# ghazalehnt/RecBole

Measured on AMD Instinct MI355X. Metric: train positives/sec (+neg) per node, higher is better.
Workload: dtype fp32; 1 GPU; C2 BPR-MF ml-20m-shape: 138,494 users x 26,745 items (incl. PAD), ~20M interactions RO_RS 0.8/0.1/0.1, embedding 128, 4 uniform negatives, 512 positives (2,048 rows) per step, dense Adam; global_batch=512, per_gpu_batch=512, train_interactions=16014928, parallelism=single, exchange_graph=True, sampler=walk (bit-exact)

## Files before the change

### include/mirec.h

```cpp
#ifndef MIREC_H
#define MIREC_H

#include <stddef.h>
#include <stdint.h>

#ifdef __cplusplus
extern "C" {
#endif

#define MIREC_ABI_VERSION 24

int mirec_abi_version(void);
const char* mirec_last_error(void);

size_t mirec_sample_walk_workspace_size(int64_t batch_keys, int64_t num);
int mirec_sample_walk(const int32_t* random_list, int64_t L, int64_t* pr_dev,
                      const int64_t* keys, int64_t n_keys, int64_t batch_keys,
                      int64_t n_batches, int64_t num,
                      const int64_t* used_ptr, const int32_t* used_cols,
                      const uint32_t* used_bits, int64_t n_bits,
                      int64_t n_key_space, int reject,
                      int64_t* out, int64_t out_stride, int32_t* status_dev,
                      void* ws, size_t ws_bytes, void* stream);

int mirec_sample_walk_segments(const int32_t* random_list, int64_t L, int64_t* pr_dev,
// ... 227 lines not shown
                                const uint32_t* const* masks, const int32_t* want,
                                const int32_t* rows_per_wave, int32_t walk_waves,
                                const float* step_consts_dev, const int32_t* step_base_dev,
                                int32_t step_off, double beta1, double beta2, double eps,
                                double weight_decay, void* stream);
int mirec_row_bitmap(const int64_t* keys, int64_t n_keys, int64_t n_rows, uint32_t* bitmap,
                     void* stream);
#define MIREC_FIRST_NOT_READ (-1)
int mirec_first_read(const int32_t* uniq, const int32_t* n_uniq, int64_t n_batches, int64_t per,
                     int64_t n_rows, int32_t* first, void* stream);
int mirec_adam_flush_first_f32(const mirec_adam_table* tables, int32_t n_tables, int32_t d,
                               const int32_t* const* first, const int32_t* rows_per_wave,
                               const float* step_consts_dev, const int32_t* step_base_dev,
                               int32_t step_off, double beta1, double beta2, double eps,
                               double weight_decay, void* stream);
int mirec_bpr_adam_step_f32(const mirec_adam_table* tables, const int64_t* n_max_uniq,
                            int32_t d, const int64_t* items, int64_t Bc, int32_t T, float gamma,
                            float grad_scale, float* loss_k, const int32_t* u_rec,
                            const int32_t* u_crec, const int32_t* i_rec, const int32_t* i_crec,
                            float* u_part, int32_t* u_join, float* i_part, int32_t* i_join,
                            const float* step_consts_dev, const int32_t* step_base_dev,
                            int32_t step_off, double beta1, double beta2, double eps,
                            double weight_decay, void* stream);
int mirec_step_records(const int64_t* user_keys, const int64_t* item_keys, int64_t n_batches,
                       int64_t Bc, int32_t T, int64_t n_users, int64_t n_items,
                       const int32_t* u_perm, const int32_t* u_uniq, const int32_t* u_seg,
                       const int32_t* u_nu, const int32_t* i_perm, const int32_t* i_uniq,
                       const int32_t* i_seg, const int32_t* i_nu, int32_t* u_rec,
                       int32_t* u_crec, int32_t* i_rec, int32_t* i_crec, int32_t* u_ahead,
                       int32_t* u_nah, int32_t* i_ahead, int32_t* i_nah, void* stream);
// ... 376 lines not shown
```

### recbole_amd/_native.py

```python
from __future__ import annotations

import ctypes
import os
from ctypes import c_double, c_float, c_int, c_int32, c_int64, c_size_t, c_void_p, c_char_p

import torch

_HERE = os.path.dirname(os.path.abspath(__file__))
LIB_PATH = os.environ.get("MIREC_LIB", os.path.join(_HERE, "_lib", "libmirec.so"))

_P = c_void_p


class RowsRef(ctypes.Structure):
    _fields_ = [('lo', _P), ('hi', _P), ('split', c_int64)]


class RowsLd(ctypes.Structure):
    _fields_ = [('lo', _P), ('hi', _P), ('split', c_int64), ('ld', c_int64)]


class SpmmEpilogue(ctypes.Structure):
    _fields_ = [('add', RowsRef), ('add_scale', c_float), ('y', RowsRef), ('acc_in', RowsRef),
                ('acc_out', RowsRef), ('acc_scale', c_float)]
# ... 170 lines not shown
                                             c_int32, c_double, c_double, c_double, c_double,
                                             _P]),
    "mirec_adam_flush_f32": (c_int, [ctypes.POINTER(AdamTable), c_int32, c_int32, _P, _P,
                                     c_int32, c_double, c_double, c_double, c_double, _P]),
    "mirec_adam_flush_rows_f32": (c_int, [ctypes.POINTER(AdamTable), c_int32, c_int32, _P, _P,
                                          _P, c_int32, c_double, c_double, c_double, c_double,
                                          _P]),
    "mirec_adam_flush_masked_f32": (c_int, [ctypes.POINTER(AdamTable), c_int32, c_int32, _P, _P,
                                            _P, c_int32, _P, _P, c_int32, c_double, c_double,
                                            c_double, c_double, _P]),
    "mirec_row_bitmap": (c_int, [_P, c_int64, c_int64, _P, _P]),
    "mirec_first_read": (c_int, [_P, _P, c_int64, c_int64, c_int64, _P, _P]),
    "mirec_adam_flush_first_f32": (c_int, [ctypes.POINTER(AdamTable), c_int32, c_int32, _P, _P,
                                           _P, _P, c_int32, c_double, c_double, c_double,
                                           c_double, _P]),
    "mirec_bpr_adam_step_f32": (c_int, [ctypes.POINTER(AdamTable), _P, c_int32, _P, c_int64,
                                        c_int32, ctypes.c_float, ctypes.c_float, _P, _P, _P,
                                        _P, _P, _P, _P, _P, _P, _P, _P, c_int32, c_double,
                                        c_double, c_double, c_double, _P]),
    "mirec_step_record_ints": (c_int64, [c_int64]),
    "mirec_colsum_multi_f32": (c_int, [_P, _P, _P, _P, c_int32, _P]),
    "mirec_offset_keys": (c_int, [_P, _P, c_int32, c_int64, _P, _P]),
    "mirec_bpr_fwd_bwd_at_ids_f32": (c_int, [_P, c_int64, c_int32, _P, _P, _P, c_int64, c_int32,
                                             ctypes.c_float, ctypes.c_float, _P, _P, _P]),
    "mirec_chunk_group_fits": (c_int, [c_int64, c_int32, c_int64, c_int64, c_int32]),
    "mirec_chunk_group": (c_int, [_P, _P, c_int64, c_int64, c_int32, c_int64, c_int64] + [_P] * 16
                          + [_P]),
    "mirec_step_records": (c_int, [_P, _P, c_int64, c_int64, c_int32, c_int64, c_int64, _P, _P,
                                   _P, _P, _P, _P, _P, _P, _P, _P, _P, _P, _P, _P, _P, _P,
                                   _P]),
# ... 95 lines not shown
                                      _P, _P, _P]),
    "mirec_ngcf_grid_cap": (c_int32, [c_int32]),
    "mirec_ngcf_shape_ok": (c_int, [c_int32, c_int32]),
    "mirec_ngcf_layer_fwd_f32": (c_int, [ctypes.POINTER(RowsLd), _P, c_int64, c_int32, c_int32,
                                         _P, _P, _P, _P, ctypes.POINTER(RowsLd), _P, _P, c_float,
                                         ctypes.c_uint64, _P, _P, _P]),
    "mirec_ngcf_layer_bwd_f32": (c_int, [ctypes.POINTER(RowsLd), ctypes.POINTER(RowsLd), _P,
                                         c_int64, c_int32, c_int32, _P, _P,
                                         ctypes.POINTER(RowsLd), _P, ctypes.POINTER(RowsLd), _P,
                                         _P, _P, c_float, ctypes.c_uint64, _P, _P, _P]),
    "mirec_ngcf_wgrad_splits": (c_int32, [c_int64]),
    "mirec_ngcf_wgrad_f32": (c_int, [_P, ctypes.POINTER(RowsLd), _P, c_int64, c_int32, c_int32,
                                     _P, _P]),
}

ABI_VERSION = 24


class NativeError(RuntimeError):
    pass


_lib = None


def lib():
    global _lib
    if _lib is not None:
        return _lib
    if not os.path.exists(LIB_PATH):
        raise NativeError(
# ... 32 lines not shown
```

### recbole_amd/csrc/adam.hip

```cpp

#include "adam_core.h"

namespace mirec {

template <int D>
__global__ __launch_bounds__(kAdamThreads) void adam_multi_kernel(
    const AdamTables tabs, const float* __restrict__ consts, const int32_t* __restrict__ step_base,
    int step_off, AdamConsts k) {
  constexpr int VPR = D / 4;
  constexpr int RPP = kAdamThreads / VPR;
  static_assert(kAdamThreads % VPR == 0, "row width");
  __shared__ int32_t slot[kAdamRows];
  __shared__ int32_t s_range[2];

  const int si = segment_of(tabs, blockIdx.x);
  const mirec_adam_table& T = tabs.t[si];
  float* __restrict__ P = T.p;
  float* __restrict__ M = T.m;
  float* __restrict__ V = T.v;
  const int32_t* __restrict__ uniq = T.uniq;

  const int64_t lo = ((int64_t)blockIdx.x - tabs.block_start[si]) * kAdamRows;
  const int64_t hi = min(T.n_rows, lo + kAdamRows);
  if (threadIdx.x < kAdamRows) slot[threadIdx.x] = -1;
// ... 261 lines not shown
    const int f = ff.first[si][r0 + lane];
    if (f > kFirstNotRead) {
      target = base + f;
      raw = T.last[r0 + lane];
    }
  }
  uint64_t todo = __ballot(min(raw, target) < target);
  while (todo) {
    const int i = __builtin_ctzll(todo);
    todo &= todo - 1;
    flush_row<D>(T, r0 + i, __builtin_amdgcn_readfirstlane(__shfl(raw, i, 64)),
                 __builtin_amdgcn_readfirstlane(__shfl(target, i, 64)), lane, consts, k);
  }
}

constexpr int kWalkRows = 32;

template <int D>
__global__ __launch_bounds__(64) void adam_flush_walk_kernel(
    const AdamTables tabs, const float* __restrict__ consts, const int32_t* __restrict__ step_base,
    int step_off, AdamConsts k, FlushMasks masks) {
  const int lane = threadIdx.x;
  const int target = step_base[0] + step_off;
  for (int si = 0; si < tabs.n_seg; ++si) {
    const mirec_adam_table& T = tabs.t[si];
    const uint32_t* __restrict__ bits = masks.bits[si];
    const uint32_t flip = masks.want[si] ? 0u : ~0u;
    const int64_t groups = (T.n_rows + kWalkRows - 1) / kWalkRows;
    for (int64_t g = blockIdx.x; g < groups; g += gridDim.x) {
      const int64_t r0 = g * kWalkRows;
      const uint32_t sel = bits ? (bits[g] ^ flip) : ~0u;
      int raw = kZeroState;
      if (lane < kWalkRows && r0 + lane < T.n_rows && ((sel >> lane) & 1u))
        raw = T.last[r0 + lane];
      uint64_t todo = __ballot(flush_needs(T, raw, target));
      while (todo) {
        const int i = __builtin_ctzll(todo);
        todo &= todo - 1;
        flush_row<D>(T, r0 + i, __shfl(raw, i, 64), target, lane, consts, k);
      }
    }
  }
}

}

using namespace mirec;

namespace {

enum class Sched { kStreamed, kDeferred, kFlush, kDeferredPair };

int launch_adam(Sched sched, const mirec_adam_table* tables, int32_t n_tables,
                const int64_t* n_max_uniq, int32_t d, const float* consts,
                const int32_t* step_base, int32_t step_off, double beta1, double beta2,
// ... 36 lines not shown
        set_error("%s: rows per wave %d of table %d not in [1, 64]", what, flush_rows[q], q);
        return -1;
      }
      fr.r[q] = flush_rows[q];
    }
    scan = true;
  }
  const bool walk = masks && walk_waves > 0;
  if (masks && (sched != Sched::kFlush || d < 64 || (!scan && !walk))) {
    set_error("%s: a masked flush needs d >= 64 and rows per wave or a wave count", what);
    return -1;
  }
  FlushMasks fm;
  memset(&fm, 0, sizeof(fm));
  if (masks) fm = *masks;
  if (firsts && (sched != Sched::kFlush || !scan || masks)) {
    set_error("%s: per-row targets need the flush with rows per wave and no mask", what);
    return -1;
  }
  FlushFirst ff;
  memset(&ff, 0, sizeof(ff));
  if (firsts) ff = *firsts;
  int scan_threads = kAdamThreads;
  if (scan && !walk) {
    int64_t waves = 0;
    for (int q = 0; q < n_tables; ++q)
      if (tables[q].n_rows > 0) waves += (tables[q].n_rows + fr.r[q] - 1) / fr.r[q];
    if (waves <= kScanOneWaveMax) scan_threads = 64;
  }
  AdamTables tabs;
  memset(&tabs, 0, sizeof(tabs));
  const bool deferred = sched == Sched::kDeferred;
// ... 48 lines not shown
    }
  }
  (void)VPR;
  for (int q = tabs.n_seg; q <= 2 * kMaxTables; ++q) tabs.block_start[q] = blocks;
  if (blocks == 0) return 0;
  AdamConsts k;
  k.omb1 = (float)(1.0 - beta1);
  k.omb1m1 = k.omb1 - 1.0f;
  k.lerp_small = fabsf(k.omb1) < 0.5f;
  k.b2 = (float)beta2;
  k.omb2 = (float)(1.0 - beta2);
  k.eps = (float)eps;
  k.wd = (float)weight_decay;
  const dim3 grd((unsigned)blocks), blk(kAdamThreads);
  hipStream_t st = (hipStream_t)stream;
#define MIREC_ADAM_SCHED(DD)                                                                 \
  case DD:                                                                                   \
    if (sched == Sched::kStreamed)                                                           \
      hipLaunchKernelGGL(adam_multi_kernel<DD>, grd, blk, 0, st, tabs, consts, step_base,    \
                         step_off, k);                                                       \
    else if (deferred && pair)                                                               \
      hipLaunchKernelGGL((dvec == 2 ? adam_deferred_pair_kernel<DD, float2>                  \
                                    : adam_deferred_pair_kernel<DD, float>),                 \
                         grd, dim3(deferred_block(1)), 0, st, tabs, consts, step_base,       \
                         step_off, k);                                                       \
    else if (deferred)                                                                       \
      hipLaunchKernelGGL((dvec == 4 ? adam_deferred_kernel<DD, float4>                       \
                          : dvec == 2 ? adam_deferred_kernel<DD, float2>                     \
                                      : adam_deferred_kernel<DD, float>),                    \
                         grd, dim3(deferred_block(DD / dvec)), 0, st, tabs, consts,          \
                         step_base, step_off, k);                                            \
    else if (DD >= 64 && walk)                                                               \
      hipLaunchKernelGGL(adam_flush_walk_kernel<(DD >= 64 ? DD : 64)>, grd, dim3(64), 0, st,   \
                         tabs, consts, step_base, step_off, k, fm);                          \
    else if (DD >= 64 && scan && firsts)                                                     \
      hipLaunchKernelGGL(adam_flush_first_kernel<(DD >= 64 ? DD : 64)>, grd,                 \
                         dim3(scan_threads), 0, st, tabs, consts, step_base, step_off, k,    \
                         fr, ff);                                                            \
    else if (DD >= 64 && scan && masks)                                                      \
      hipLaunchKernelGGL((adam_flush_scan_kernel<(DD >= 64 ? DD : 64), true>), grd,          \
                         dim3(scan_threads), 0, st, tabs, consts, step_base, step_off, k,    \
                         fr, fm);                                                            \
    else if (DD >= 64 && scan)                                                               \
      hipLaunchKernelGGL((adam_flush_scan_kernel<(DD >= 64 ? DD : 64), false>), grd,         \
                         dim3(scan_threads), 0, st, tabs, consts, step_base, step_off, k,    \
                         fr, fm);                                                            \
    else if (DD >= 64)                                                                       \
      hipLaunchKernelGGL(adam_flush_row_kernel<(DD >= 64 ? DD : 64)>, grd,                   \
                         dim3(kFlushRowThreads), 0, st, tabs,                                \
// ... 144 lines not shown
  FlushFirst ff;
  memset(&ff, 0, sizeof(ff));
  int n = 0;
  for (int q = 0; q < n_tables; ++q) {
    if (!first[q]) continue;
    sel[n] = tables[q];
    rows[n] = rows_per_wave[q];
    ff.first[n] = first[q];
    ++n;
  }
  if (n == 0) return 0;
  return launch_adam(Sched::kFlush, sel, n, nullptr, d, step_consts_dev, step_base_dev, step_off,
                     beta1, beta2, eps, weight_decay, stream, what, rows, nullptr, 0, &ff);
}

extern "C" int mirec_adam_sparse_grad_f32(float* p, float* m, float* v, int64_t n_rows,
                                          int32_t d, const float* rows, const int32_t* perm,
                                          const int32_t* uniq, const int32_t* seg,
                                          const int32_t* n_uniq_dev, int64_t n_max_uniq,
                                          const float* dense_grad, const float* step_consts_dev,
                                          const int32_t* step_idx_dev, double beta1,
                                          double beta2, double eps, double weight_decay,
                                          void* stream) {
  (void)n_max_uniq;
  if (n_rows == 0) return 0;
  mirec_adam_table t;
  memset(&t, 0, sizeof(t));
  t.p = p; t.m = m; t.v = v; t.n_rows = n_rows;
  t.rows = rows; t.perm = perm; t.uniq = uniq; t.seg = seg; t.n_uniq = n_uniq_dev;
  t.dense_grad = dense_grad;
// ... 152 lines not shown
```

### recbole_amd/csrc/common.h

```cpp
#pragma once
#include <hip/hip_runtime.h>
#include <stdint.h>
#include <stdio.h>
#include <string.h>
#include "../../include/mirec.h"

namespace mirec {

void set_error(const char* fmt, ...);

inline int hip_status(hipError_t e, const char* what) {
  if (e == hipSuccess) return 0;
  set_error("%s: %s", what, hipGetErrorString(e));
  return -(1000 + (int)e);
}

inline int launch_status(const char* what) {
  return hip_status(hipGetLastError(), what);
}

constexpr int kMaxDev = 16;

inline int current_device() {
  int dev = -1;
// ... 25 lines not shown
  if (rc) return rc;
  int n = 1;
  if (per_cu) {
    if (hipOccupancyMaxActiveBlocksPerMultiprocessor(&n, (const void*)kern, threads, lds) !=
        hipSuccess) {
      (void)hipGetLastError();
      n = 1;
    }
    n = n < 1 ? 1 : (n > 4 ? 4 : n);
    *per_cu = n;
  }
  if (dev >= 0) cache[dev] = n;
  return 0;
}

constexpr int kWave = 64;

__device__ __forceinline__ float wave_sum(float x) {
#pragma unroll
  for (int off = 32; off > 0; off >>= 1) x += __shfl_xor(x, off, 64);
  return x;
}

__device__ __forceinline__ int wave_sum_i(int x) {
#pragma unroll
  for (int off = 32; off > 0; off >>= 1) x += __shfl_xor(x, off, 64);
  return x;
}

__device__ __forceinline__ int wave_inclusive_scan(int v) {
// ... 42 lines not shown
```

### recbole_amd/ops.py

```python
from __future__ import annotations

import ctypes

import numpy as np
import torch

from recbole_amd._native import NativeError, check, lib, ptr, stream_handle

KERNEL_EVENTS = None


class timed_launch(object):

    def __init__(self, name):
        self.name = name
        self.ev = None

    def __enter__(self):
        if KERNEL_EVENTS is not None and self.name in KERNEL_EVENTS:
            self.ev = (torch.cuda.Event(enable_timing=True), torch.cuda.Event(enable_timing=True))
            self.ev[0].record()
        return self

    def __exit__(self, *exc):
# ... 769 lines not shown
        nm = (ctypes.c_int64 * len(tables))(*n_max_uniq)
        rc = lib().mirec_adam_deferred_f32(tables, len(tables), nm, d, *args)
    elif schedule == "deferred_pair":
        nm = (ctypes.c_int64 * 2)(*n_max_uniq)
        rc = lib().mirec_adam_deferred_pair_f32(tables, nm, d, *args)
    elif schedule == "flush" and flush_rows is not None:
        rpw = (ctypes.c_int32 * len(tables))(*flush_rows)
        rc = lib().mirec_adam_flush_rows_f32(tables, len(tables), d, rpw, *args)
    elif schedule == "flush":
        rc = lib().mirec_adam_flush_f32(tables, len(tables), d, *args)
    else:
        raise ValueError(f"unknown schedule {schedule!r}")
    check(rc, f"adam_multi[{schedule}]")


_TICKETS = {}


def finish_ticket(device, tag=''):
    key = (str(device), tag)
    t = _TICKETS.get(key)
    if t is None:
        t = _TICKETS[key] = torch.zeros(1, dtype=torch.int32, device=device)
    return t


def chunk_finish(loss_k, n: int, stride: int, n_steps: int, denom: float, loss_hist, step_base):
    _dev(loss_k, torch.float32, "loss_k")
    _dev(step_base, torch.int32, "step_base")
    rc = lib().mirec_chunk_finish(ptr(loss_k), n, stride, n_steps, float(denom), ptr(loss_hist),
# ... 710 lines not shown
```

### recbole_amd/trainer/chunk_plan.py

```python
from __future__ import annotations

import bisect
import math


def plan_chunks(n, Bg, C, ramp, cuts=(), ramps=(0,)):
    full = n // Bg
    bounds = sorted({0, full} | {int(c) for c in cuts if 0 < int(c) < full})
    ramp_at = {int(r) for r in ramps}
    out = []
    for lo, hi in zip(bounds[:-1], bounds[1:]):
        ri = 0 if lo in ramp_at else len(ramp)
        b0 = lo
        while b0 < hi:
            size = ramp[ri] if ri < len(ramp) else C
            ri += 1
            nb = min(size, C, hi - b0)
            out.append((b0, nb, Bg))
            b0 += nb
    if n % Bg:
        out.append((full, 1, n % Bg))
    return out


# ... 49 lines not shown
    on = bool(enabled and fused_step and use_graph and adam_mode == 'deferred')
    return [bool(on and Bc == Bg and nb >= min_steps) for _, nb, Bc in plan]


def advance_rows(nb, Bg, times, n_rows, max_rows):
    out = []
    for per, rows in zip((Bg, (1 + times) * Bg), n_rows):
        frac = min(1.0, nb * per / max(rows, 1))
        r = 1
        while r * 2 <= max_rows and r * 2 * frac <= 1.0:
            r *= 2
        out.append(r)
    return tuple(out)


def chunk_of(plan, b):
    return max(bisect.bisect_right(plan, (b, math.inf)) - 1, 0)
```

### recbole_amd/trainer/fused.py

```python
from __future__ import annotations

import ctypes
import math
import os
from types import SimpleNamespace

import numpy as np
import torch

from recbole_amd import ops
from recbole_amd._native import AdamTable, ChunkPrep, check, lib
from recbole_amd.trainer import chunk_plan
from recbole_amd.trainer.exchange import ExchangeLayout

REC_CONTRIB = 8
ADAM_MODES = ('deferred', 'streamed')


_PREP_STREAMS = {}


def _prep_streams_for(dev, n=2):
    key = (str(dev), n)
    got = _PREP_STREAMS.get(key)
# ... 43 lines not shown
    def __init__(self, C, B, T, G, dev, ahead, tab=None):
        Bg = G * B
        KI = (1 + T) * Bg
        self.user_keys = torch.empty(C * Bg, dtype=torch.int64, device=dev)
        self.item_keys = torch.empty(C * KI, dtype=torch.int64, device=dev)
        self.lu = self.li = None
        if G > 1:
            self.lu = torch.empty(C * B, dtype=torch.int64, device=dev)
            self.li = torch.empty(C * (1 + T) * B, dtype=torch.int64, device=dev)
        self.tab = tab or [_Lists(C, per, dev, ahead) for per in (Bg, KI)]
        self.records = None
        self.bitmap = None
        self.first = None
        self.bg_done = None
        self.bg_busy = False
        self.prep = None
        self.ready, self.walked, self.free = (torch.cuda.Event() for _ in range(3))
        cur = torch.cuda.current_stream(dev)
        for ev in (self.ready, self.walked, self.free):
            ev.record(cur)
        self.free_recorded = False
        self.group_pending = False
        self.ready_on_model = False
        self.chunk = None
        self.graphs = {}


class FusedBPRTrainStep(object):

    CHUNK = 64
    SLOTS = 3
    RAMP = (8, 16, 32)
    FLUSH_EVERY = 64
    FLUSH_SPARSE_MAX_ROWS = 8
    MAIN_FIRST = os.environ.get('MIREC_MAIN_FIRST', '1') != '0'
    SPEC_WALK = os.environ.get('MIREC_SPEC_WALK', '1') != '0'
    BG_FLUSH = os.environ.get('MIREC_BG_FLUSH', '1') != '0'
    BG_WAVES = int(os.environ.get('MIREC_BG_WAVES', '1536'))
    BG_MIN_STEPS = 32
    CHUNK_ADVANCE = os.environ.get('MIREC_CHUNK_ADVANCE', '1') != '0'
    ADV_MIN_STEPS = 32

    def __init__(self, model, optimizer, train_data, chunk=None, use_graph=True,
                 adam_mode='deferred', dist=None, fused_step=None):
        if adam_mode not in ADAM_MODES:
            raise ValueError(f'adam_mode must be one of {ADAM_MODES}, got {adam_mode!r}')
        self.model = model
        self.opt = optimizer
        self.data = train_data
        (self.pU, self.nU), (self.pI, self.nI) = model.fused_embedding_tables()
        self.device = self.pU.device
        self.B = train_data.step
        self.times = train_data.times
        self.uid_field = train_data.uid_field
        self.iid_field = train_data.iid_field
        self.C = chunk or self.CHUNK
# ... 28 lines not shown
        self.loss_hist = torch.zeros(1, dtype=torch.float32, device=dev)
        self.consts = torch.zeros(4, dtype=torch.float32, device=dev)
        self.step_idx = torch.zeros(1, dtype=torch.int32, device=dev)
        self.ticket = torch.zeros(1, dtype=torch.int32, device=dev)
        self.kernel_events = None
        self.kernel_uniq = []
        self.n_eager_steps = 0
        self._rec_w = {}
        self._spec_buf = self._spec_stats = None
        self._gs_R = self._gs = None
        self._users = self._items = None
        self.n_batches = 0
        self._plan, self._flags, self._flush_at = [], [], set()
        self._bg = []
        self._adv = []
        self._bg_pending = None
        self._bg_mark = torch.cuda.Event()
        self._bg_mark.record(torch.cuda.current_stream(dev))
        self._busy0 = None
        self._batches_enqueued = 0
        self._current = True
        self._next_chunk = self._next_group = self._prep_limit = 0
        self._cur = None
        self._last_walked = None
        self._deferred_waits = []
        self._urgent = False
        self._late_top_up = None
        self.opt._ensure_state(self.pU)
        self.opt._ensure_state(self.pI)
        self._tables = (AdamTable * 2)()
# ... 12 lines not shown
        if deferred:
            self.lastU = torch.zeros(self.nU, dtype=torch.int32, device=dev)
            self.lastI = torch.zeros(self.nI, dtype=torch.int32, device=dev)
        self.pU_alt = torch.empty_like(self.pU.data) if self.fused_step else None
        self.pI_alt = torch.empty_like(self.pI.data) if self.fused_step else None
        self._step_scratch = None
        if self.fused_step:
            for sl in self.slots:
                sl.records = [torch.empty(self.C * w, dtype=torch.int32, device=dev)
                              for w in self._rec_ints(self.Bg)]
                sl.bitmap = torch.zeros((self.nU + 31) // 32, dtype=torch.int32, device=dev)
                sl.first = [torch.full((n,), -1, dtype=torch.int32, device=dev)
                            for n in (self.nU, self.nI)]
                sl.bg_done = torch.cuda.Event()
                sl.bg_done.record(torch.cuda.current_stream(dev))
            self._step_scratch = ops.step_scratch(self.Bg, T, d, dev)
        self._n_max = (ctypes.c_int64 * 2)(self.Bg, (1 + T) * self.Bg)
        self._fill_tables()

    def _flush_rows(self, b_end):
        return chunk_plan.flush_rows(b_end, self.Bg, self.times, self.adam_mode, self.d,
                                     [t.n_rows for t in self._tables], self._busy0,
                                     self.FLUSH_SPARSE_MAX_ROWS)

    def _chunk_of(self, b):
        return chunk_plan.chunk_of(self._plan, b)

    def _dp_slice(self, Bc):
        return self.G > 1 and Bc == self.Bg

# ... 75 lines not shown
    def _apply_deferred_waits(self):
        for st, ev in self._deferred_waits:
            st.wait_event(ev)
        self._deferred_waits = []

    def _prepare_group(self, slot):
        self._apply_deferred_waits()
        self.group_stream.wait_event(slot.walked)
        self._group_on(slot, self.group_stream)

    def _group_on(self, slot, st):
        check(lib().mirec_prepare_chunk_group(ctypes.byref(slot.prep), st.cuda_stream),
              'mirec_prepare_chunk_group')
        b0, nb, Bc = slot.chunk
        if slot.bitmap is not None and self._bg[self._chunk_of(b0)]:
            check(lib().mirec_row_bitmap(slot.user_keys.data_ptr(), nb * Bc, self.nU,
                                         slot.bitmap.data_ptr(), st.cuda_stream),
                  'mirec_row_bitmap')
        if slot.first is not None and self._adv[self._chunk_of(b0)]:
            for l, per, n, first in zip(slot.tab, (Bc, (1 + self.times) * Bc),
                                        (self.nU, self.nI), slot.first):
                check(lib().mirec_first_read(l.uniq.data_ptr(), l.nu.data_ptr(), nb, per, n,
                                             first.data_ptr(), st.cuda_stream),
                      'mirec_first_read')
        slot.ready.record(st)
        slot.group_pending = False

    def _chunk_prep(self, slot):
        if slot.prep is not None:
            return slot.prep
# ... 213 lines not shown
        t = (AdamTable * 2)()
        ctypes.memmove(t, self._tables, ctypes.sizeof(t))
        self._point_tables(t, [SimpleNamespace(perm=uniq, uniq=uniq, seg=uniq, nu=self.zero_i32,
                                               ahead=uniq, nah=n)
                               for uniq, n in self._entry_lists(slot)], 0, (0, 0), True)
        t[0].rows = t[1].rows = self.xbuf.data_ptr()
        self._adam(stream, -1, t, 'ahead')

    def _advance(self, slot, stream, nb):
        rows = chunk_plan.advance_rows(nb, self.Bg, self.times, (self.nU, self.nI),
                                       self.FLUSH_SPARSE_MAX_ROWS)
        self._launch('advance', stream, 'mirec_adam_flush_first_f32', self._tables, 2, self.d,
                     (ctypes.c_void_p * 2)(*[f.data_ptr() for f in slot.first]),
                     (ctypes.c_int32 * 2)(*rows), *self._sched(0))

    def _grad_scale(self, Bc):
        R = Bc * self.times
        if self._gs_R != R:
            self._gs_R = R
            self._gs = float(np.float32(1.0) / np.float32(R))
        return self._gs

    def _graph_for(self, slot, nb, entry, flush, masked=False, advance=False):
        key = (nb, entry, flush, masked, advance)
        g = slot.graphs.get(key)
        if g is None:
            g = torch.cuda.CUDAGraph()
            cap = torch.cuda.Stream(device=self.device)
            cap.wait_stream(torch.cuda.current_stream(self.device))
            with torch.cuda.graph(g, stream=cap):
                if entry and not advance:
                    self._entry(slot, cap)
                for c in range(nb):
                    self._step(slot, c, self.Bg, cap, c, c + 1 < nb)
                self._finish(0, nb, self.Bg, cap)
                if flush and masked:
                    self._flush_masked(cap, slot, chunk_plan.masked_flush_rows(
                        flush, nb, self.Bg, self.nU, self.FLUSH_SPARSE_MAX_ROWS))
                elif flush:
                    self._flush(cap, flush)
            torch.cuda.current_stream(self.device).wait_stream(cap)
            slot.graphs[key] = g
        return g

    def _capture_variants(self):
        S = len(self.slots)
        variants = sorted({(k % S, n, e, f, bg, adv) for k, ((_, n, Bc), (e, f), bg, adv) in
                           enumerate(zip(self._plan, self._flags, self._bg, self._adv))
                           if Bc == self.Bg},
                          key=lambda v: (v[0], v[1], v[2], repr(v[3]), v[4], v[5]))
        for k, n, e, f, bg, adv in variants:
            self._graph_for(self.slots[k], n, e, f, bg, adv)

    def begin_epoch(self, cuts=(), hold_prep_from=None, flush_at=()):
        self._await_background(torch.cuda.current_stream(self.device))
        data = self.data
        if data.shuffle:
            data._shuffle()
        inter = data.dataset.inter_feat
        self._users = inter[self.uid_field]
        self._items = inter[self.iid_field]
        if not self._users.is_cuda:
            raise RuntimeError('fused train step needs the train table on the GPU')
        self.n_batches = nb = math.ceil(self._users.numel() / self.Bg)
        table = self.opt.step_constants(self.opt.n_steps + 1, max(nb, 1)).reshape(-1)
        ptrs = [(t.p, t.m, t.v) for t in self._tables]
        self._fill_tables()
# ... 20 lines not shown
            self.pU_alt.copy_(self.pU.data)
            self.pI_alt.copy_(self.pI.data)
        ramps = (0,) if hold_prep_from is None else (0, int(hold_prep_from))
        self._plan = chunk_plan.plan_chunks(self._users.numel(), self.Bg, self.C, self.RAMP,
                                            cuts, ramps)
        self._flush_at = set(int(b) for b in flush_at)
        self._flags = chunk_plan.chunk_flags(self._plan, self.Bg, self.FLUSH_EVERY,
                                             self._flush_at, self.times, self.adam_mode, self.d,
                                             n_rows, self._busy0, self.FLUSH_SPARSE_MAX_ROWS)
        self._bg = chunk_plan.bg_flush_chunks(self._plan, self._flags, self.Bg, self.adam_mode,
                                              self.fused_step, self.use_graph,
                                              self.BG_MIN_STEPS, self.BG_FLUSH)
        self._adv = chunk_plan.advance_chunks(self._plan, self.Bg, self.adam_mode,
                                              self.fused_step, self.use_graph,
                                              self.ADV_MIN_STEPS, self.CHUNK_ADVANCE)
        if self.use_graph:
            self._capture_variants()
        self.prep_stream.wait_stream(torch.cuda.current_stream(self.device))
        self._last_walked = None
        self._deferred_waits, self._urgent, self._late_top_up = [], False, None
        self._next_chunk = 0
        self._next_group = 0
        self._prep_limit = (len(self._plan) if hold_prep_from is None
                            else self._chunk_of(hold_prep_from))
        self._cur = None
        for s in self.slots:
            s.free_recorded = False
            if not self._dp_slice(self.Bg):
                self._chunk_prep(s)
        for _ in range(len(self.slots)):
# ... 56 lines not shown

    def run_batches(self, b_start, b_end):
        stream = torch.cuda.current_stream(self.device)
        b = b_start
        while b < b_end:
            k = self._chunk_of(b)
            b0, nb, Bc = self._plan[k]
            entry, flush = self._flags[k]
            self._await_background(stream)
            self._enter_chunk(k, stream)
            slot = self.slots[k % len(self.slots)]
            c0, c1 = b - b0, min(nb, b_end - b0)
            key = (nb, entry, flush, self._bg[k], self._adv[k])
            if (self.use_graph and c0 == 0 and c1 == nb and Bc == self.Bg
                    and self.kernel_events is None and key in slot.graphs):
                if self._adv[k]:
                    self._advance(slot, stream, nb)
                if chunk_plan.bg_flush_now(self._bg[k], c0, c1, nb, key in slot.graphs,
                                           self.kernel_events is not None):
                    self._flush_background(slot, b0 + nb, stream)
                slot.graphs[key].replay()
                self._current = flush
            else:
                self.n_eager_steps += c1 - c0
                if c0 == 0 and entry:
                    self._entry(slot, stream)
                for c in range(c0, c1):
                    self._step(slot, c, Bc, stream, 0, c + 1 < nb)
                    self._finish(c, 1, Bc, stream)
                self._current = False
                if c1 == nb and flush:
                    self._flush(stream, flush)
                    self._current = True
            if self._late_top_up == k:
                self._late_top_up = None
                self._urgent = True
                self._top_up_prep(k)
                self._urgent = False
            self._issue_groups(k + len(self.slots))
            b = b0 + c1
            self._batches_enqueued = b

    def _top_up_prep(self, k):
        lim = min(len(self._plan), self._prep_limit, k + len(self.slots))
        while self._next_chunk < lim:
            self._issue_prep()

    def sync_params(self):
        self._await_background(torch.cuda.current_stream(self.device))
        if not self._current:
            self._flush(torch.cuda.current_stream(self.device),
                        self._flush_rows(self._batches_enqueued))
            self._current = True

    def end_epoch(self, n_done=None):
        n_done = self.n_batches if n_done is None else n_done
        stream = torch.cuda.current_stream(self.device)
        self._await_background(stream)
        stream.wait_stream(self.prep_stream)
        stream.wait_stream(self.group_stream)
        self.sync_params()
        self.opt.advance(n_done)
        self.data.pr = 0
        self.data.sampler.check_status()
# ... 23 lines not shown
```

Baseline: 29.45 million positives/s.

## Fuse chunk-close masked flush with next chunk's advance flush; ticket-based walk flush

Adds a boundary Adam flush kernel that closes the previous chunk's masked rows and applies the next chunk's first-read catch-up in one pass. It captures 'open' graph variants that skip the trailing masked flush so the next chunk can fuse it in. The walk flush kernel now takes work from an atomic ticket in 8-row units instead of a fixed grid stride, and the default background wave count is lowered. The boundary path is off by default (MIREC_BOUNDARY=0), so by default only the ticket walk and the wave count change take effect.

```diff
diff --git a/include/mirec.h b/include/mirec.h
--- a/include/mirec.h
+++ b/include/mirec.h
@@ -8,7 +8,7 @@
 extern "C" {
 #endif
 
-#define MIREC_ABI_VERSION 24
+#define MIREC_ABI_VERSION 25
 
 int mirec_abi_version(void);
 const char* mirec_last_error(void);
@@ -266,6 +266,11 @@
                                const float* step_consts_dev, const int32_t* step_base_dev,
                                int32_t step_off, double beta1, double beta2, double eps,
                                double weight_decay, void* stream);
+int mirec_adam_flush_boundary_f32(const mirec_adam_table* tables, int32_t n_tables, int32_t d,
+                                  const uint32_t* const* masks, const int32_t* const* first,
+                                  const int32_t* rows_per_wave, const float* step_consts_dev,
+                                  const int32_t* step_base_dev, int32_t step_off, double beta1,
+                                  double beta2, double eps, double weight_decay, void* stream);
 int mirec_bpr_adam_step_f32(const mirec_adam_table* tables, const int64_t* n_max_uniq,
                             int32_t d, const int64_t* items, int64_t Bc, int32_t T, float gamma,
                             float grad_scale, float* loss_k, const int32_t* u_rec,
diff --git a/recbole_amd/_native.py b/recbole_amd/_native.py
--- a/recbole_amd/_native.py
+++ b/recbole_amd/_native.py
@@ -208,6 +208,9 @@
     "mirec_adam_flush_first_f32": (c_int, [ctypes.POINTER(AdamTable), c_int32, c_int32, _P, _P,
                                            _P, _P, c_int32, c_double, c_double, c_double,
                                            c_double, _P]),
+    "mirec_adam_flush_boundary_f32": (c_int, [ctypes.POINTER(AdamTable), c_int32, c_int32, _P,
+                                              _P, _P, _P, _P, c_int32, c_double, c_double,
+                                              c_double, c_double, _P]),
     "mirec_bpr_adam_step_f32": (c_int, [ctypes.POINTER(AdamTable), _P, c_int32, _P, c_int64,
                                         c_int32, ctypes.c_float, ctypes.c_float, _P, _P, _P,
                                         _P, _P, _P, _P, _P, _P, _P, _P, c_int32, c_double,
@@ -333,7 +336,7 @@
                                      _P, _P]),
 }
 
-ABI_VERSION = 24
+ABI_VERSION = 25
 
 
 class NativeError(RuntimeError):
diff --git a/recbole_amd/csrc/adam.hip b/recbole_amd/csrc/adam.hip
--- a/recbole_amd/csrc/adam.hip
+++ b/recbole_amd/csrc/adam.hip
@@ -299,31 +299,74 @@
   }
 }
 
-constexpr int kWalkRows = 32;
+template <int D>
+__global__ __launch_bounds__(kAdamThreads) void adam_flush_boundary_kernel(
+    const AdamTables tabs, const float* __restrict__ consts, const int32_t* __restrict__ step_base,
+    int step_off, AdamConsts k, FlushRows rows_per_wave, FlushMasks masks, FlushFirst ff) {
+  const int si = segment_of(tabs, blockIdx.x);
+  const mirec_adam_table& T = tabs.t[si];
+  const int R = rows_per_wave.r[si];
+  const int lane = threadIdx.x & 63;
+  const int64_t r0 =
+      (((int64_t)blockIdx.x - tabs.block_start[si]) * (blockDim.x >> 6) + (threadIdx.x >> 6)) * R;
+  if (r0 >= T.n_rows) return;
+  const int base = step_base[0] + step_off;
+  int raw = kZeroState, target = base;
+  bool close = false;
+  if (lane < R && r0 + lane < T.n_rows) {
+    close = mask_selects(masks.bits[si], masks.want[si], r0 + lane);
+    const int f = ff.first[si] ? ff.first[si][r0 + lane] : kFirstNotRead;
+    if (f > kFirstNotRead) target = base + f;
+    if (close || f > kFirstNotRead) raw = T.last[r0 + lane];
+  }
+  uint64_t todo = __ballot(close ? flush_needs(T, raw, target) : min(raw, target) < target);
+  while (todo) {
+    const int i = __builtin_ctzll(todo);
+    todo &= todo - 1;
+    flush_row<D>(T, r0 + i, __builtin_amdgcn_readfirstlane(__shfl(raw, i, 64)),
+                 __builtin_amdgcn_readfirstlane(__shfl(target, i, 64)), lane, consts, k);
+  }
+}
+
+#ifndef MIREC_WALK_UNIT
+#define MIREC_WALK_UNIT 8
+#endif
+constexpr int kWalkUnit = MIREC_WALK_UNIT;
+static_assert(kWalkUnit >= 1 && kWalkUnit <= 32 && (kWalkUnit & (kWalkUnit - 1)) == 0,
+              "a walk unit is a power of two inside one 32-row bitmap word");
+struct WalkUnits {
+  uint32_t end[kMaxTables];
+};
 
 template <int D>
 __global__ __launch_bounds__(64) void adam_flush_walk_kernel(
     const AdamTables tabs, const float* __restrict__ consts, const int32_t* __restrict__ step_base,
-    int step_off, AdamConsts k, FlushMasks masks) {
+    int step_off, AdamConsts k, FlushMasks masks, WalkUnits units, uint32_t* __restrict__ ticket) {
   const int lane = threadIdx.x;
   const int target = step_base[0] + step_off;
-  for (int si = 0; si < tabs.n_seg; ++si) {
+  const uint32_t total = units.end[tabs.n_seg - 1];
+  for (;;) {
+    uint32_t u = 0;
+    if (lane == 0)
+      u = __hip_atomic_fetch_add(ticket, 1u, __ATOMIC_RELAXED, __HIP_MEMORY_SCOPE_AGENT);
+    u = __builtin_amdgcn_readfirstlane(u);
+    if (u >= total) break;
+    int si = 0;
+    uint32_t first = 0;
+    while (u >= units.end[si]) first = units.end[si++];
     const mirec_adam_table& T = tabs.t[si];
     const uint32_t* __restrict__ bits = masks.bits[si];
     const uint32_t flip = masks.want[si] ? 0u : ~0u;
-    const int64_t groups = (T.n_rows + kWalkRows - 1) / kWalkRows;
-    for (int64_t g = blockIdx.x; g < groups; g += gridDim.x) {
-      const int64_t r0 = g * kWalkRows;
-      const uint32_t sel = bits ? (bits[g] ^ flip) : ~0u;
-      int raw = kZeroState;
-      if (lane < kWalkRows && r0 + lane < T.n_rows && ((sel >> lane) & 1u))
-        raw = T.last[r0 + lane];
-      uint64_t todo = __ballot(flush_needs(T, raw, target));
-      while (todo) {
-        const int i = __builtin_ctzll(todo);
-        todo &= todo - 1;
-        flush_row<D>(T, r0 + i, __shfl(raw, i, 64), target, lane, consts, k);
-      }
+    const int64_t r0 = (int64_t)(u - first) * kWalkUnit;
+    const uint32_t sel = bits ? ((bits[r0 >> 5] ^ flip) >> (r0 & 31)) : ~0u;
+    int raw = kZeroState;
+    if (lane < kWalkUnit && r0 + lane < T.n_rows && ((sel >> lane) & 1u))
+      raw = T.last[r0 + lane];
+    uint64_t todo = __ballot(flush_needs(T, raw, target));
+    while (todo) {
+      const int i = __builtin_ctzll(todo);
+      todo &= todo - 1;
+      flush_row<D>(T, r0 + i, __shfl(raw, i, 64), target, lane, consts, k);
     }
   }
 }
@@ -390,8 +433,8 @@
   FlushMasks fm;
   memset(&fm, 0, sizeof(fm));
   if (masks) fm = *masks;
-  if (firsts && (sched != Sched::kFlush || !scan || masks)) {
-    set_error("%s: per-row targets need the flush with rows per wave and no mask", what);
+  if (firsts && (sched != Sched::kFlush || !scan || walk)) {
+    set_error("%s: per-row targets need the flush with rows per wave", what);
     return -1;
   }
   FlushFirst ff;
@@ -470,6 +513,22 @@
   k.wd = (float)weight_decay;
   const dim3 grd((unsigned)blocks), blk(kAdamThreads);
   hipStream_t st = (hipStream_t)stream;
+  WalkUnits wu;
+  memset(&wu, 0, sizeof(wu));
+  uint32_t* ticket = nullptr;
+  if (walk) {
+    uint64_t end = 0;
+    for (int q = 0; q < kMaxTables; ++q) {
+      if (q < n_tables) end += (uint64_t)((tables[q].n_rows + kWalkUnit - 1) / kWalkUnit);
+      if (end + (uint64_t)walk_waves >= (1ull << 32)) {
+        set_error("%s: too many rows for the walk form's 32-bit ticket", what);
+        return -1;
+      }
+      wu.end[q] = (uint32_t)end;
+    }
+    const int rc = launch_ticket(st, &ticket, what);
+    if (rc) return rc;
+  }
 #define MIREC_ADAM_SCHED(DD)                                                                 \
   case DD:                                                                                   \
     if (sched == Sched::kStreamed)                                                           \
@@ -488,7 +547,11 @@
                          step_base, step_off, k);                                            \
     else if (DD >= 64 && walk)                                                               \
       hipLaunchKernelGGL(adam_flush_walk_kernel<(DD >= 64 ? DD : 64)>, grd, dim3(64), 0, st,   \
-                         tabs, consts, step_base, step_off, k, fm);                          \
+                         tabs, consts, step_base, step_off, k, fm, wu, ticket);              \
+    else if (DD >= 64 && scan && firsts && masks)                                            \
+      hipLaunchKernelGGL(adam_flush_boundary_kernel<(DD >= 64 ? DD : 64)>, grd,              \
+                         dim3(scan_threads), 0, st, tabs, consts, step_base, step_off, k,    \
+                         fr, fm, ff);                                                        \
     else if (DD >= 64 && scan && firsts)                                                     \
       hipLaunchKernelGGL(adam_flush_first_kernel<(DD >= 64 ? DD : 64)>, grd,                 \
                          dim3(scan_threads), 0, st, tabs, consts, step_base, step_off, k,    \
@@ -663,6 +726,33 @@
                      beta1, beta2, eps, weight_decay, stream, what, rows, nullptr, 0, &ff);
 }
 
+extern "C" int mirec_adam_flush_boundary_f32(const mirec_adam_table* tables, int32_t n_tables,
+                                             int32_t d, const uint32_t* const* masks,
+                                             const int32_t* const* first,
+                                             const int32_t* rows_per_wave,
+                                             const float* step_consts_dev,
+                                             const int32_t* step_base_dev, int32_t step_off,
+                                             double beta1, double beta2, double eps,
+                                             double weight_decay, void* stream) {
+  const char* what = "mirec_adam_flush_boundary_f32";
+  if (!tables || n_tables < 1 || n_tables > kMaxTables || !first || !rows_per_wave) {
+    set_error("%s: bad arguments (first-read arrays and rows per wave, per table)", what);
+    return -1;
+  }
+  FlushMasks fm;
+  FlushFirst ff;
+  memset(&fm, 0, sizeof(fm));
+  memset(&ff, 0, sizeof(ff));
+  for (int q = 0; q < n_tables; ++q) {
+    fm.bits[q] = masks ? masks[q] : nullptr;
+    fm.want[q] = 1;
+    ff.first[q] = first[q];
+  }
+  return launch_adam(Sched::kFlush, tables, n_tables, nullptr, d, step_consts_dev, step_base_dev,
+                     step_off, beta1, beta2, eps, weight_decay, stream, what, rows_per_wave, &fm,
+                     0, &ff);
+}
+
 extern "C" int mirec_adam_sparse_grad_f32(float* p, float* m, float* v, int64_t n_rows,
                                           int32_t d, const float* rows, const int32_t* perm,
                                           const int32_t* uniq, const int32_t* seg,
diff --git a/recbole_amd/csrc/common.h b/recbole_amd/csrc/common.h
--- a/recbole_amd/csrc/common.h
+++ b/recbole_amd/csrc/common.h
@@ -3,6 +3,9 @@
 #include <stdint.h>
 #include <stdio.h>
 #include <string.h>
+#include <mutex>
+#include <utility>
+#include <vector>
 #include "../../include/mirec.h"
 
 namespace mirec {
@@ -63,6 +66,52 @@
   return 0;
 }
 
+constexpr int kTicketSlab = 1024;
+
+inline int launch_ticket(hipStream_t stream, uint32_t** word, const char* what) {
+  struct Dev {
+    std::vector<std::pair<hipStream_t, uint32_t*>> by_stream;
+    uint32_t* slab = nullptr;
+    int used = 0;
+  };
+  static std::mutex mu;
+  static Dev devs[kMaxDev];
+  const int dev = current_device();
+  if (dev < 0) {
+    set_error("%s: no ticket word for this device (index past %d)", what, kMaxDev);
+    return -1;
+  }
+  hipStreamCaptureStatus cap = hipStreamCaptureStatusNone;
+  if (hipStreamIsCapturing(stream, &cap) != hipSuccess) {
+    (void)hipGetLastError();
+    cap = hipStreamCaptureStatusNone;
+  }
+  uint32_t* w = nullptr;
+  {
+    std::lock_guard<std::mutex> lock(mu);
+    Dev& D = devs[dev];
+    if (cap == hipStreamCaptureStatusNone)
+      for (const auto& e : D.by_stream)
+        if (e.first == stream) w = e.second;
+    if (!w) {
+      if (!D.slab || D.used == kTicketSlab) {
+        hipStreamCaptureMode mode = hipStreamCaptureModeRelaxed;
+        (void)hipThreadExchangeStreamCaptureMode(&mode);
+        void* p = nullptr;
+        const hipError_t e = hipMalloc(&p, kTicketSlab * sizeof(uint32_t));
+        (void)hipThreadExchangeStreamCaptureMode(&mode);
+        if (e != hipSuccess) return hip_status(e, what);
+        D.slab = static_cast<uint32_t*>(p);
+        D.used = 0;
+      }
+      w = D.slab + D.used++;
+      if (cap == hipStreamCaptureStatusNone) D.by_stream.emplace_back(stream, w);
+    }
+  }
+  *word = w;
+  return hip_status(hipMemsetAsync(w, 0, sizeof(uint32_t), stream), what);
+}
+
 constexpr int kWave = 64;
 
 __device__ __forceinline__ float wave_sum(float x) {
diff --git a/recbole_amd/ops.py b/recbole_amd/ops.py
--- a/recbole_amd/ops.py
+++ b/recbole_amd/ops.py
@@ -807,6 +807,22 @@
     check(rc, f"adam_multi[{schedule}]")
 
 
+def adam_flush_boundary(tables, d: int, masks, first, rows_per_wave, step_consts, step_base,
+                        step_off: int = 0, beta1=0.9, beta2=0.999, eps=1e-8, weight_decay=0.0):
+    import ctypes
+    n = len(tables)
+    _dev(step_consts, torch.float32, "step_consts")
+    _dev(step_base, torch.int32, "step_base")
+    mp = (ctypes.c_void_p * n)(*[ptr(_dev(m, torch.int32, "mask")) if m is not None else None
+                                 for m in masks])
+    fp = (ctypes.c_void_p * n)(*[ptr(_dev(f, torch.int32, "first")) if f is not None else None
+                                 for f in first])
+    rc = lib().mirec_adam_flush_boundary_f32(
+        tables, n, d, mp, fp, (ctypes.c_int32 * n)(*rows_per_wave), ptr(step_consts),
+        ptr(step_base), step_off, beta1, beta2, eps, weight_decay, stream_handle())
+    check(rc, "mirec_adam_flush_boundary_f32")
+
+
 _TICKETS = {}
 
 
diff --git a/recbole_amd/trainer/chunk_plan.py b/recbole_amd/trainer/chunk_plan.py
--- a/recbole_amd/trainer/chunk_plan.py
+++ b/recbole_amd/trainer/chunk_plan.py
@@ -87,5 +87,24 @@
     return tuple(out)
 
 
+def boundary_chunks(plan, flags, bg, adv, flush_at, enabled=True):
+    cut = {int(b) for b in flush_at}
+    out = [False] * len(plan)
+    for k in range(1, len(plan)):
+        b0, end = plan[k][0], plan[k - 1][0] + plan[k - 1][1]
+        out[k] = bool(enabled and bg[k - 1] and flags[k - 1][1] and adv[k] and b0 == end
+                      and b0 not in cut)
+    return out
+
+
+def boundary_now(planned_next, whole_graph, next_end, b_end, next_graph_ready, timed_kernels):
+    return bool(planned_next and whole_graph and next_end <= b_end and next_graph_ready
+                and not timed_kernels)
+
+
+def boundary_rows(close_rows, advance_rows_):
+    return tuple(min(a, b) for a, b in zip(close_rows, advance_rows_))
+
+
 def chunk_of(plan, b):
     return max(bisect.bisect_right(plan, (b, math.inf)) - 1, 0)
diff --git a/recbole_amd/trainer/fused.py b/recbole_amd/trainer/fused.py
--- a/recbole_amd/trainer/fused.py
+++ b/recbole_amd/trainer/fused.py
@@ -81,6 +81,8 @@
         self.first = None
         self.bg_done = None
         self.bg_busy = False
+        self.close_done = None
+        self.close_busy = False
         self.prep = None
         self.ready, self.walked, self.free = (torch.cuda.Event() for _ in range(3))
         cur = torch.cuda.current_stream(dev)
@@ -103,10 +105,11 @@
     MAIN_FIRST = os.environ.get('MIREC_MAIN_FIRST', '1') != '0'
     SPEC_WALK = os.environ.get('MIREC_SPEC_WALK', '1') != '0'
     BG_FLUSH = os.environ.get('MIREC_BG_FLUSH', '1') != '0'
-    BG_WAVES = int(os.environ.get('MIREC_BG_WAVES', '1536'))
+    BG_WAVES = int(os.environ.get('MIREC_BG_WAVES', '1024'))
     BG_MIN_STEPS = 32
     CHUNK_ADVANCE = os.environ.get('MIREC_CHUNK_ADVANCE', '1') != '0'
     ADV_MIN_STEPS = 32
+    BOUNDARY = os.environ.get('MIREC_BOUNDARY', '0') != '0'
 
     def __init__(self, model, optimizer, train_data, chunk=None, use_graph=True,
                  adam_mode='deferred', dist=None, fused_step=None):
@@ -165,6 +168,8 @@
         self._plan, self._flags, self._flush_at = [], [], set()
         self._bg = []
         self._adv = []
+        self._bnd = []
+        self._open = None
         self._bg_pending = None
         self._bg_mark = torch.cuda.Event()
         self._bg_mark.record(torch.cuda.current_stream(dev))
@@ -207,6 +212,8 @@
                             for n in (self.nU, self.nI)]
                 sl.bg_done = torch.cuda.Event()
                 sl.bg_done.record(torch.cuda.current_stream(dev))
+                sl.close_done = torch.cuda.Event()
+                sl.close_done.record(torch.cuda.current_stream(dev))
             self._step_scratch = ops.step_scratch(self.Bg, T, d, dev)
         self._n_max = (ctypes.c_int64 * 2)(self.Bg, (1 + T) * self.Bg)
         self._fill_tables()
@@ -312,6 +319,9 @@
               'mirec_prepare_chunk_group')
         b0, nb, Bc = slot.chunk
         if slot.bitmap is not None and self._bg[self._chunk_of(b0)]:
+            if slot.close_busy:
+                st.wait_event(slot.close_done)
+                slot.close_busy = False
             check(lib().mirec_row_bitmap(slot.user_keys.data_ptr(), nb * Bc, self.nU,
                                          slot.bitmap.data_ptr(), st.cuda_stream),
                   'mirec_row_bitmap')
@@ -555,6 +565,28 @@
                      (ctypes.c_void_p * 2)(*[f.data_ptr() for f in slot.first]),
                      (ctypes.c_int32 * 2)(*rows), *self._sched(0))
 
+    def _boundary(self, prev, slot, stream, nb):
+        _, prev_nb, flush = self._open
+        rows = chunk_plan.boundary_rows(
+            chunk_plan.masked_flush_rows(flush, prev_nb, self.Bg, self.nU,
+                                         self.FLUSH_SPARSE_MAX_ROWS),
+            chunk_plan.advance_rows(nb, self.Bg, self.times, (self.nU, self.nI),
+                                    self.FLUSH_SPARSE_MAX_ROWS))
+        self._launch('boundary', stream, 'mirec_adam_flush_boundary_f32', self._tables, 2,
+                     self.d, (ctypes.c_void_p * 2)(prev.bitmap.data_ptr(), None),
+                     (ctypes.c_void_p * 2)(*[f.data_ptr() for f in slot.first]),
+                     (ctypes.c_int32 * 2)(*rows), *self._sched(0))
+        prev.close_done.record(stream)
+        prev.close_busy = True
+        self._open = None
+
+    def _close_open(self, stream):
+        if self._open is not None:
+            prev, prev_nb, flush = self._open
+            self._flush_masked(stream, prev, chunk_plan.masked_flush_rows(
+                flush, prev_nb, self.Bg, self.nU, self.FLUSH_SPARSE_MAX_ROWS))
+            self._open = None
+
     def _grad_scale(self, Bc):
         R = Bc * self.times
         if self._gs_R != R:
@@ -562,8 +594,8 @@
             self._gs = float(np.float32(1.0) / np.float32(R))
         return self._gs
 
-    def _graph_for(self, slot, nb, entry, flush, masked=False, advance=False):
-        key = (nb, entry, flush, masked, advance)
+    def _graph_for(self, slot, nb, entry, flush, masked=False, advance=False, close=True):
+        key = (nb, entry, flush, masked, advance) + (() if close else ('open',))
         g = slot.graphs.get(key)
         if g is None:
             g = torch.cuda.CUDAGraph()
@@ -575,7 +607,9 @@
                 for c in range(nb):
                     self._step(slot, c, self.Bg, cap, c, c + 1 < nb)
                 self._finish(0, nb, self.Bg, cap)
-                if flush and masked:
+                if not close:
+                    pass
+                elif flush and masked:
                     self._flush_masked(cap, slot, chunk_plan.masked_flush_rows(
                         flush, nb, self.Bg, self.nU, self.FLUSH_SPARSE_MAX_ROWS))
                 elif flush:
@@ -592,6 +626,9 @@
                           key=lambda v: (v[0], v[1], v[2], repr(v[3]), v[4], v[5]))
         for k, n, e, f, bg, adv in variants:
             self._graph_for(self.slots[k], n, e, f, bg, adv)
+        for k, ((_, n, _), (e, f)) in enumerate(zip(self._plan, self._flags)):
+            if k + 1 < len(self._plan) and self._bnd[k + 1]:
+                self._graph_for(self.slots[k % S], n, e, f, self._bg[k], self._adv[k], close=False)
 
     def begin_epoch(self, cuts=(), hold_prep_from=None, flush_at=()):
         self._await_background(torch.cuda.current_stream(self.device))
@@ -642,6 +679,9 @@
         self._adv = chunk_plan.advance_chunks(self._plan, self.Bg, self.adam_mode,
                                               self.fused_step, self.use_graph,
                                               self.ADV_MIN_STEPS, self.CHUNK_ADVANCE)
+        self._bnd = chunk_plan.boundary_chunks(self._plan, self._flags, self._bg, self._adv,
+                                               self._flush_at, self.BOUNDARY)
+        self._open = None
         if self.use_graph:
             self._capture_variants()
         self.prep_stream.wait_stream(torch.cuda.current_stream(self.device))
@@ -728,14 +768,28 @@
             key = (nb, entry, flush, self._bg[k], self._adv[k])
             if (self.use_graph and c0 == 0 and c1 == nb and Bc == self.Bg
                     and self.kernel_events is None and key in slot.graphs):
-                if self._adv[k]:
+                if self._open is not None:
+                    self._boundary(self._open[0], slot, stream, nb)
+                elif self._adv[k]:
                     self._advance(slot, stream, nb)
-                if chunk_plan.bg_flush_now(self._bg[k], c0, c1, nb, key in slot.graphs,
-                                           self.kernel_events is not None):
+                bg_now = chunk_plan.bg_flush_now(self._bg[k], c0, c1, nb, key in slot.graphs,
+                                                 self.kernel_events is not None)
+                if bg_now:
                     self._flush_background(slot, b0 + nb, stream)
-                slot.graphs[key].replay()
-                self._current = flush
+                nxt = self._plan[k + 1] if k + 1 < len(self._plan) else None
+                okey = key + ('open',)
+                if nxt is not None and chunk_plan.boundary_now(
+                        self._bnd[k + 1] and okey in slot.graphs, bg_now, nxt[0] + nxt[1], b_end,
+                        (nxt[1],) + self._flags[k + 1] + (self._bg[k + 1], self._adv[k + 1])
+                        in self.slots[(k + 1) % len(self.slots)].graphs, False):
+                    slot.graphs[okey].replay()
+                    self._open = (slot, nb, flush)
+                    self._current = False
+                else:
+                    slot.graphs[key].replay()
+                    self._current = flush
             else:
+                self._close_open(stream)
                 self.n_eager_steps += c1 - c0
                 if c0 == 0 and entry:
                     self._entry(slot, stream)
@@ -762,6 +816,7 @@
 
     def sync_params(self):
         self._await_background(torch.cuda.current_stream(self.device))
+        self._open = None
         if not self._current:
             self._flush(torch.cuda.current_stream(self.device),
                         self._flush_rows(self._batches_enqueued))
```

After: 29.30 million positives/s. About the same (-0.5%).
